# apache/incubator-predictionio

Measured on NVIDIA H100. Metric: ALS iterations/sec, higher is better.
Workload: dtype f32

## Files before the change

### incubator-predictionio_b200/csrc/als_pair_kernel.cuh

```cuda
#pragma once
#include <cuda_fp16.h>
#include <cuda_runtime.h>
#include <stdint.h>

#include "als_kernels.cuh"
#include "als_lockstep.cuh"

namespace pio {
namespace pr {

constexpr int KP = 64;
constexpr int CH = 8;
constexpr int RSTR = KP;
constexpr int NSTAGE = 4;
constexpr int STAGE = CH * RSTR;
constexpr int NTILE = 20;
using LL = LsLayout<KP>;
constexpr int SLOT_STRIDE = LL::STRIDE;
constexpr int VSTR = 80;
constexpr int PART_FLOATS = LL::SIZE + KP;
static_assert(NSTAGE * STAGE <= SLOT_STRIDE, "the staging ring lives in the second slot");
static_assert(NSTAGE % 2 == 0, "a loop step consumes two stages");
constexpr int W_BVEC = 2 * SLOT_STRIDE;
constexpr int W_COL = W_BVEC + 2 * VSTR;
constexpr int W_MVAL = W_COL + 2 * VSTR;
constexpr int W_FLOATS = W_MVAL + NSTAGE * CH + 8;
constexpr size_t smem_bytes(int warps) { return sizeof(float) * (size_t)W_FLOATS * warps; }

__device__ __forceinline__ int split_exponent(float vmax) {
  if (!(vmax > 0.f)) return 0;
  if (isinf(vmax)) return -63;
  int x;
  frexpf(vmax, &x);
  const int e = 15 - x;
  return e < -63 ? -63 : e > 63 ? 63 : e;
}
__device__ __forceinline__ float pow2f(int e) { return __int_as_float((127 + e) << 23); }

__global__ void __launch_bounds__(256) abs_max_kernel(const float* __restrict__ x, long long n, unsigned* out) {
  float m = 0.f;
  const long long stride = (long long)gridDim.x * blockDim.x;
  const long long i0 = (long long)blockIdx.x * blockDim.x + threadIdx.x;
  long long tail = 0;
  if ((reinterpret_cast<uintptr_t>(x) & 15) == 0) {
    const long long n4 = n >> 2;
    for (long long i = i0; i < n4; i += stride) {
      const float4 v = __ldg(reinterpret_cast<const float4*>(x) + i);
      m = fmaxf(m, fmaxf(fmaxf(fabsf(v.x), fabsf(v.y)), fmaxf(fabsf(v.z), fabsf(v.w))));
    }
    tail = 4 * n4;
  }
  for (long long i = tail + i0; i < n; i += stride) m = fmaxf(m, fabsf(__ldg(x + i)));
#pragma unroll
  for (int o = 16; o > 0; o >>= 1) m = fmaxf(m, __shfl_xor_sync(0xffffffffu, m, o));
  if ((threadIdx.x & 31) == 0) atomicMax(out, __float_as_uint(m));
}

__device__ __forceinline__ uint64_t pack2(uint32_t x, uint32_t y) {
  uint64_t r;
  asm("mov.b64 %0, {%1, %2};" : "=l"(r) : "r"(x), "r"(y));
  return r;
}
__device__ __forceinline__ void mma_f16_p(float (&d)[4], const uint32_t (&a)[4], uint64_t b) {
  asm volatile(
      "{\n .reg .b32 b0, b1;\n mov.b64 {b0, b1}, %8;\n"
      "mma.sync.aligned.m16n8k16.row.col.f32.f16.f16.f32 {%0,%1,%2,%3}, {%4,%5,%6,%7}, {b0,b1}, {%0,%1,%2,%3};\n}\n"
      : "+f"(d[0]), "+f"(d[1]), "+f"(d[2]), "+f"(d[3])
      : "r"(a[0]), "r"(a[1]), "r"(a[2]), "r"(a[3]), "l"(b));
}
__device__ __forceinline__ void mma_f16_zp(float (&d)[4], const uint32_t (&a)[4], uint64_t b) {
  asm volatile(
      "{\n .reg .b32 b0, b1;\n mov.b64 {b0, b1}, %4;\n"
      "mma.sync.aligned.m16n8k16.row.col.f32.f16.f16.f32 {%0,%1,%2,%3}, {%5,%6,%7,%8}, {b0,b1}, {%9,%9,%9,%9};\n}\n"
      : "=f"(d[0]), "=f"(d[1]), "=f"(d[2]), "=f"(d[3])
      : "l"(b), "r"(a[0]), "r"(a[1]), "r"(a[2]), "r"(a[3]), "f"(0.f));
}

__device__ __forceinline__ void split2(float a, float b, uint32_t& hi, uint32_t& lo) {
  const __half2 h = __floats2half2_rn(a, b);
  const float2 hf = __half22float2(h);
  const __half2 l = __floats2half2_rn(__fsub_rn(a, hf.x), __fsub_rn(b, hf.y));
  hi = *reinterpret_cast<const uint32_t*>(&h);
  lo = *reinterpret_cast<const uint32_t*>(&l);
}

template <bool IMPLICIT>
__device__ __forceinline__ void accumulate_row(const SolveParams& p, long long beg, long long end, float s, float unscale,
                                               const float* __restrict__ yty, float* ring, float* mval, float* slot,
                                               float* bv) {
  const int lane = threadIdx.x & 31;
  const int g = lane >> 2, t = lane & 3;
  const int nchunks = 2 * (int)((end - beg + 2 * CH - 1) / (2 * CH));
  const int prow = lane >> 4, psl = lane & 15;

  int nidx;
  float nval;
  auto prefetch_meta = [&](int c) {
    const long long e = beg + (long long)c * CH + (lane & 15);
    nidx = (c < nchunks && e < end) ? __ldg(p.idx + e) : -1;
    nval = (lane < 2 * CH && c < nchunks && e < end) ? __ldg(p.val + e) : 0.f;
  };
  auto issue = [&](int c) {
    if (c < nchunks) {
#pragma unroll
      for (int h = 0; h < 2; ++h) {
        float* sbuf = ring + ((c + h) % NSTAGE) * STAGE;
#pragma unroll
        for (int j = 0; j < 4; ++j) {
          const int r = 2 * j + prow;
          const int src = __shfl_sync(0xffffffffu, nidx, CH * h + r);
          float4* d4 = reinterpret_cast<float4*>(sbuf + r * RSTR + ((psl * 4) ^ (8 * r)));
          if (src >= 0) cp_async16(d4, p.src + (size_t)src * KP + psl * 4);
          else *d4 = make_float4(0.f, 0.f, 0.f, 0.f);
        }
      }
      if (lane < 2 * CH) mval[(c % NSTAGE) * CH + lane] = nval;
    }
    cp_async_commit();
  };

  float acc[NTILE][4];
#pragma unroll
  for (int i = 0; i < NTILE; ++i)
#pragma unroll
    for (int e = 0; e < 4; ++e) acc[i][e] = 0.f;
  float pb[4][2];
#pragma unroll
  for (int i = 0; i < 4; ++i) pb[i][0] = pb[i][1] = 0.f;

  int xo[4];
#pragma unroll
  for (int q = 0; q < 4; ++q) xo[q] = g + 8 * (q ^ t);

  prefetch_meta(0);
  issue(0);
  prefetch_meta(2);

#pragma unroll 1
  for (int c = 0; c < nchunks; c += 2) {
    cp_async_wait<0>();
    __syncwarp();
    issue(c + 2);
    prefetch_meta(c + 4);
    const float* XA = ring + (c % NSTAGE) * STAGE + t * RSTR;
    const float* XB = XA + STAGE;
    const float* mv = mval + (c % NSTAGE) * CH;
    float wb[4], sc[4];
    {
      const float r[4] = {mv[t], mv[t + 4], mv[CH + t], mv[CH + t + 4]};
#pragma unroll
      for (int q = 0; q < 4; ++q) {
        wb[q] = r[q];
        sc[q] = s;
        if (IMPLICIT) {
          const float c1 = p.alpha * fabsf(r[q]);
          sc[q] = __fmul_rn(sqrtf(c1), s);
          wb[q] = r[q] > 0.f ? 1.f + c1 : 0.f;
        }
      }
    }
    uint32_t hi[4][4], lo[4][4];
#pragma unroll
    for (int i = 0; i < 4; ++i) {
#pragma unroll
      for (int e = 0; e < 2; ++e) {
        const int q = 2 * i + e;
        const int c0 = xo[q & 3] + 32 * (q >> 2), c4 = 4 * RSTR + xo[q & 3] + 32 * (1 - (q >> 2));
        const float a0 = XA[c0], a4 = XA[c4], b0 = XB[c0], b4 = XB[c4];
        pb[i][e] = fmaf(wb[0], a0, pb[i][e]);
        pb[i][e] = fmaf(wb[1], a4, pb[i][e]);
        pb[i][e] = fmaf(wb[2], b0, pb[i][e]);
        pb[i][e] = fmaf(wb[3], b4, pb[i][e]);
        split2(__fmul_rn(a0, sc[0]), __fmul_rn(a4, sc[1]), hi[i][e], lo[i][e]);
        split2(__fmul_rn(b0, sc[2]), __fmul_rn(b4, sc[3]), hi[i][e + 2], lo[i][e + 2]);
      }
    }
#pragma unroll
    for (int j = 0; j < 8; ++j) {
      const int bi = j >> 1, be = j & 1;
      const uint64_t bh = pack2(hi[bi][be], hi[bi][be + 2]), bl = pack2(lo[bi][be], lo[bi][be + 2]);
#pragma unroll
      for (int i = bi; i < 4; ++i) {
        const int tile = i * (i + 1) + j;
        float d[4];
        mma_f16_zp(d, lo[i], bh);
        mma_f16_p(d, hi[i], bl);
        mma_f16_p(d, hi[i], bh);
        acc[tile][0] += d[0];
        acc[tile][1] += d[1];
        acc[tile][2] += d[2];
        acc[tile][3] += d[3];
      }
    }
  }
  cp_async_wait<0>();
  __syncwarp();

#pragma unroll
  for (int i = 0; i < 4; ++i)
#pragma unroll
    for (int e = 0; e < 2; ++e) {
      float v = pb[i][e];
      v += __shfl_xor_sync(0xffffffffu, v, 1);
      v += __shfl_xor_sync(0xffffffffu, v, 2);
      if (t == 0) bv[16 * i + 8 * e + g] = v;
    }
  {
    const float* yl = yty ? yty + g * KP + 2 * t : nullptr;
    int tile = 0;
#pragma unroll
    for (int i = 0; i < 4; ++i) {
#pragma unroll
      for (int j = 0; j <= 2 * i + 1; ++j, ++tile) {
        const int cb = j >> 1;
        const int cc = 8 * (j & 1) + 2 * t;
        float d0 = acc[tile][0] * unscale, d1 = acc[tile][1] * unscale;
        float d2 = acc[tile][2] * unscale, d3 = acc[tile][3] * unscale;
        if (yl) {
          const float2 y0 = __ldg(reinterpret_cast<const float2*>(yl + 16 * i * KP + 8 * j));
          const float2 y1 = __ldg(reinterpret_cast<const float2*>(yl + (16 * i + 8) * KP + 8 * j));
          d0 += y0.x; d1 += y0.y;
          d2 += y1.x; d3 += y1.y;
        }
        if (cb < i) {
          *reinterpret_cast<float2*>(slot + LL::offd(i, cb, g, cc)) = make_float2(d0, d1);
          *reinterpret_cast<float2*>(slot + LL::offd(i, cb, g + 8, cc)) = make_float2(d2, d3);
        } else {
          if (cc <= g) slot[LL::diag(i, g, cc)] = d0;
          if (cc + 1 <= g) slot[LL::diag(i, g, cc + 1)] = d1;
          if (cc <= g + 8) slot[LL::diag(i, g + 8, cc)] = d2;
          if (cc + 1 <= g + 8) slot[LL::diag(i, g + 8, cc + 1)] = d3;
        }
      }
    }
  }
  __syncwarp();
}

__device__ __forceinline__ void fill_identity(float* slot, float* bv) {
  const int lane = threadIdx.x & 31;
  for (int o = lane; o < LL::SIZE; o += 32) slot[o] = 0.f;
  __syncwarp();
  for (int r = lane; r < KP; r += 32) {
    slot[LL::at(r, r)] = 1.f;
    bv[r] = 0.f;
  }
  __syncwarp();
}

template <bool IMPLICIT, int WARPS>
__global__ void __launch_bounds__(32 * WARPS, 12 / WARPS) als_solve_pair_kernel(const SolveParams p, int n_items) {
  extern __shared__ __align__(16) float smem_all[];
  const int warp = threadIdx.x >> 5;
  float* smem = smem_all + warp * W_FLOATS;
  float* slot0 = smem;
  float* slot1 = smem + SLOT_STRIDE;
  float* ring = slot1;
  float* bvec = smem + W_BVEC;
  float* colbuf = smem + W_COL;
  float* mval = smem + W_MVAL;
  const int lane = threadIdx.x & 31;
  const int grp = lane >> 4;
  const int npairs = (n_items + 1) >> 1;
  const float c1_root_max = IMPLICIT ? sqrtf(p.alpha * __uint_as_float(__ldg(p.absmax + 1))) : 1.f;
  const int e = split_exponent(__uint_as_float(__ldg(p.absmax)) * c1_root_max);
  const float s = pow2f(e), unscale = pow2f(-2 * e);

#pragma unroll 1
  for (int base = blockIdx.x * WARPS; base < npairs; base += gridDim.x * WARPS) {
    const int pair = base + warp;
    int row0 = -1, row1 = -1;
    if (pair < npairs) {
#pragma unroll 1
      for (int h = 0; h < 2; ++h) {
        const int item = 2 * pair + h;
        float* slot = h ? slot1 : slot0;
        float* bv = bvec + h * VSTR;
        if (item >= n_items) {
          fill_identity(slot, bv);
          continue;
        }
        long long beg, end;
        if (p.partial) {
          beg = p.wl_beg[item];
          end = p.wl_end[item];
        } else {
          const int r = p.row_begin + item;
          beg = p.ptr[r];
          end = p.ptr[r + 1];
          if (h) row1 = r;
          else row0 = r;
        }
        accumulate_row<IMPLICIT>(p, beg, end, s, unscale, IMPLICIT && !p.partial ? p.yty : nullptr, ring, mval, slot, bv);
        if (p.partial) {
          float* out = p.partial + (size_t)item * PART_FLOATS;
          for (int o = lane; o < LL::SIZE / 4; o += 32)
            reinterpret_cast<float4*>(out)[o] = reinterpret_cast<const float4*>(slot)[o];
          for (int o = lane; o < KP; o += 32) out[LL::SIZE + o] = bv[o];
          __syncwarp();
        }
      }
    }
    if (p.partial) continue;
    if (WARPS > 1) __syncthreads();
    if (pair < npairs) {
      const int myrow = grp ? row1 : row0;
      const int rr = myrow < 0 ? p.row_begin : myrow;
      chol_lockstep<KP>(grp ? slot1 : slot0, bvec + grp * VSTR, p.lambda * p.nreg[rr], p.k, colbuf + grp * VSTR,
                        p.dst + (size_t)(p.dst_row_offset + rr) * KP, myrow >= 0, p.fail);
      __syncwarp();
    }
  }
}

template <bool IMPLICIT>
__global__ void __launch_bounds__(32, 12) als_finish_pair_kernel(const SolveParams p, const int* __restrict__ row_part_ptr,
                                                                  int n_rows) {
  extern __shared__ __align__(16) float smem[];
  float* bvec = smem + W_BVEC;
  float* colbuf = smem + W_COL;
  const int lane = threadIdx.x & 31;
  const int grp = lane >> 4;
  const int npairs = (n_rows + 1) >> 1;
#pragma unroll 1
  for (int pair = blockIdx.x; pair < npairs; pair += gridDim.x) {
#pragma unroll 1
    for (int h = 0; h < 2; ++h) {
      const int r = 2 * pair + h;
      float* slot = smem + h * SLOT_STRIDE;
      float* bv = bvec + h * VSTR;
      if (r >= n_rows) {
        fill_identity(slot, bv);
        continue;
      }
      const int p0 = row_part_ptr[r], p1 = row_part_ptr[r + 1];
      for (int o = lane; o < PART_FLOATS / 4; o += 32) {
        float4 s = make_float4(0.f, 0.f, 0.f, 0.f);
        for (int q = p0; q < p1; ++q) {
          const float4 v = __ldg(reinterpret_cast<const float4*>(p.partial + (size_t)q * PART_FLOATS) + o);
          s.x += v.x; s.y += v.y; s.z += v.z; s.w += v.w;
        }
        if (o < LL::SIZE / 4) reinterpret_cast<float4*>(slot)[o] = s;
        else reinterpret_cast<float4*>(bv)[o - LL::SIZE / 4] = s;
      }
      __syncwarp();
      if (IMPLICIT) {
        ls_add_yty<KP>(slot, p.yty);
        __syncwarp();
      }
    }
    const int myrow = 2 * pair + grp;
    const bool valid = myrow < n_rows;
    const int rr = valid ? myrow : 0;
    chol_lockstep<KP>(smem + grp * SLOT_STRIDE, bvec + grp * VSTR, p.lambda * p.nreg[rr], p.k, colbuf + grp * VSTR,
                      p.dst + (size_t)(p.dst_row_offset + rr) * KP, valid, p.fail);
    __syncwarp();
  }
}

}
}
```

Before: 35.54.

## Stage fp16 hi/lo planes in shared memory and feed MMAs via ldmatrix

Each lane now reads its chunk rows as float4 vectors, computes the weighted b-vector sums and the hi/lo fp16 split for its own columns, then writes the hi and lo halves back over the consumed fp32 stage. The MMA A and B fragments are then loaded with ldmatrix.x4.trans from a swizzled layout. This replaces the scalar per-element shared loads and register packing of the old scheme. The intent is to cut shared-memory load instructions and bank conflicts in the Gram accumulation loop. Missing rows are zero-filled through cp.async src-size instead of a separate store. In exchange it adds extra shared stores and two warp syncs per step, plus more register pressure from the ldmatrix fragments.

```diff
diff --git a/incubator-predictionio_b200/csrc/als_pair_kernel.cuh b/incubator-predictionio_b200/csrc/als_pair_kernel.cuh
--- a/incubator-predictionio_b200/csrc/als_pair_kernel.cuh
+++ b/incubator-predictionio_b200/csrc/als_pair_kernel.cuh
@@ -14,6 +14,8 @@
 constexpr int RSTR = KP;
 constexpr int NSTAGE = 4;
 constexpr int STAGE = CH * RSTR;
+constexpr int PLANE = 2 * CH * KP * 2;
+static_assert(PLANE == STAGE * (int)sizeof(float), "a step's hi and lo planes overwrite its two fp32 stages");
 constexpr int NTILE = 20;
 using LL = LsLayout<KP>;
 constexpr int SLOT_STRIDE = LL::STRIDE;
@@ -56,24 +58,26 @@
   if ((threadIdx.x & 31) == 0) atomicMax(out, __float_as_uint(m));
 }
 
-__device__ __forceinline__ uint64_t pack2(uint32_t x, uint32_t y) {
-  uint64_t r;
-  asm("mov.b64 %0, {%1, %2};" : "=l"(r) : "r"(x), "r"(y));
-  return r;
-}
-__device__ __forceinline__ void mma_f16_p(float (&d)[4], const uint32_t (&a)[4], uint64_t b) {
-  asm volatile(
-      "{\n .reg .b32 b0, b1;\n mov.b64 {b0, b1}, %8;\n"
-      "mma.sync.aligned.m16n8k16.row.col.f32.f16.f16.f32 {%0,%1,%2,%3}, {%4,%5,%6,%7}, {b0,b1}, {%0,%1,%2,%3};\n}\n"
-      : "+f"(d[0]), "+f"(d[1]), "+f"(d[2]), "+f"(d[3])
-      : "r"(a[0]), "r"(a[1]), "r"(a[2]), "r"(a[3]), "l"(b));
-}
-__device__ __forceinline__ void mma_f16_zp(float (&d)[4], const uint32_t (&a)[4], uint64_t b) {
-  asm volatile(
-      "{\n .reg .b32 b0, b1;\n mov.b64 {b0, b1}, %4;\n"
-      "mma.sync.aligned.m16n8k16.row.col.f32.f16.f16.f32 {%0,%1,%2,%3}, {%5,%6,%7,%8}, {b0,b1}, {%9,%9,%9,%9};\n}\n"
-      : "=f"(d[0]), "=f"(d[1]), "=f"(d[2]), "=f"(d[3])
-      : "l"(b), "r"(a[0]), "r"(a[1]), "r"(a[2]), "r"(a[3]), "f"(0.f));
+__device__ __forceinline__ void mma_f16(float (&d)[4], const uint32_t (&a)[4], uint32_t b0, uint32_t b1) {
+  asm volatile("mma.sync.aligned.m16n8k16.row.col.f32.f16.f16.f32 {%0,%1,%2,%3}, {%4,%5,%6,%7}, {%8,%9}, {%0,%1,%2,%3};\n"
+               : "+f"(d[0]), "+f"(d[1]), "+f"(d[2]), "+f"(d[3])
+               : "r"(a[0]), "r"(a[1]), "r"(a[2]), "r"(a[3]), "r"(b0), "r"(b1));
+}
+__device__ __forceinline__ void mma_f16_z(float (&d)[4], const uint32_t (&a)[4], uint32_t b0, uint32_t b1) {
+  asm volatile("mma.sync.aligned.m16n8k16.row.col.f32.f16.f16.f32 {%0,%1,%2,%3}, {%4,%5,%6,%7}, {%8,%9}, {%10,%10,%10,%10};\n"
+               : "=f"(d[0]), "=f"(d[1]), "=f"(d[2]), "=f"(d[3])
+               : "r"(a[0]), "r"(a[1]), "r"(a[2]), "r"(a[3]), "r"(b0), "r"(b1), "f"(0.f));
+}
+__device__ __forceinline__ void ldsm_x4_t(uint32_t (&r)[4], uint32_t saddr) {
+  asm volatile("ldmatrix.sync.aligned.m8n8.x4.trans.shared.b16 {%0,%1,%2,%3}, [%4];\n"
+               : "=r"(r[0]), "=r"(r[1]), "=r"(r[2]), "=r"(r[3])
+               : "r"(saddr)
+               : "memory");
+}
+
+__device__ __forceinline__ void cp_async16_zfill(void* smem_dst, const void* gsrc, bool copy) {
+  const unsigned s = (unsigned)__cvta_generic_to_shared(smem_dst);
+  asm volatile("cp.async.cg.shared.global [%0], [%1], 16, %2;\n" ::"r"(s), "l"(gsrc), "r"(copy ? 16 : 0));
 }
 
 __device__ __forceinline__ void split2(float a, float b, uint32_t& hi, uint32_t& lo) {
@@ -92,6 +96,7 @@
   const int g = lane >> 2, t = lane & 3;
   const int nchunks = 2 * (int)((end - beg + 2 * CH - 1) / (2 * CH));
   const int prow = lane >> 4, psl = lane & 15;
+  auto ring_col = [](int r, int f) { return f ^ (4 * (r & 1) + 8 * (r & 2)); };
 
   int nidx;
   float nval;
@@ -109,9 +114,8 @@
         for (int j = 0; j < 4; ++j) {
           const int r = 2 * j + prow;
           const int src = __shfl_sync(0xffffffffu, nidx, CH * h + r);
-          float4* d4 = reinterpret_cast<float4*>(sbuf + r * RSTR + ((psl * 4) ^ (8 * r)));
-          if (src >= 0) cp_async16(d4, p.src + (size_t)src * KP + psl * 4);
-          else *d4 = make_float4(0.f, 0.f, 0.f, 0.f);
+          cp_async16_zfill(sbuf + r * RSTR + ring_col(r, psl * 4), p.src + (size_t)(src < 0 ? 0 : src) * KP + psl * 4,
+                           src >= 0);
         }
       }
       if (lane < 2 * CH) mval[(c % NSTAGE) * CH + lane] = nval;
@@ -124,13 +128,17 @@
   for (int i = 0; i < NTILE; ++i)
 #pragma unroll
     for (int e = 0; e < 4; ++e) acc[i][e] = 0.f;
-  float pb[4][2];
-#pragma unroll
-  for (int i = 0; i < 4; ++i) pb[i][0] = pb[i][1] = 0.f;
-
-  int xo[4];
-#pragma unroll
-  for (int q = 0; q < 4; ++q) xo[q] = g + 8 * (q ^ t);
+  float pb[8];
+#pragma unroll
+  for (int j = 0; j < 8; ++j) pb[j] = 0.f;
+
+  int wo[2];
+#pragma unroll
+  for (int e = 0; e < 2; ++e) wo[e] = (2 * t + e) * 128 + ((g ^ (2 * t + e)) << 4);
+  const int lm = lane >> 3, lr = lane & 7;
+  const uint32_t offa = (lr + 8 * (lm >> 1)) * 128 + (((lm & 1) ^ lr) << 4);
+  const uint32_t offb = (lr + 8 * (lm & 1)) * 128 + (((lm >> 1) ^ lr) << 4);
+  const uint32_t ring_s = (uint32_t)__cvta_generic_to_shared(ring);
 
   prefetch_meta(0);
   issue(0);
@@ -140,14 +148,25 @@
   for (int c = 0; c < nchunks; c += 2) {
     cp_async_wait<0>();
     __syncwarp();
+    float* X = ring + (c % NSTAGE) * STAGE;
+    const float* mv = mval + (c % NSTAGE) * CH;
+    const float r[4] = {mv[t], mv[t + 4], mv[CH + t], mv[CH + t + 4]};
+    float x[4][8];
+#pragma unroll
+    for (int q = 0; q < 4; ++q)
+#pragma unroll
+      for (int w = 0; w < 2; ++w) {
+        const float4 v = *reinterpret_cast<const float4*>(X + (q >> 1) * STAGE + (t + 4 * (q & 1)) * RSTR +
+                                                          ring_col(t, 8 * g + 4 * w));
+        x[q][4 * w] = v.x;
+        x[q][4 * w + 1] = v.y;
+        x[q][4 * w + 2] = v.z;
+        x[q][4 * w + 3] = v.w;
+      }
     issue(c + 2);
     prefetch_meta(c + 4);
-    const float* XA = ring + (c % NSTAGE) * STAGE + t * RSTR;
-    const float* XB = XA + STAGE;
-    const float* mv = mval + (c % NSTAGE) * CH;
     float wb[4], sc[4];
     {
-      const float r[4] = {mv[t], mv[t + 4], mv[CH + t], mv[CH + t + 4]};
 #pragma unroll
       for (int q = 0; q < 4; ++q) {
         wb[q] = r[q];
@@ -160,36 +179,55 @@
       }
     }
     uint32_t hi[4][4], lo[4][4];
+    {
+#pragma unroll
+      for (int j = 0; j < 8; ++j)
+#pragma unroll
+        for (int q = 0; q < 4; ++q) pb[j] = fmaf(wb[q], x[q][j], pb[j]);
+#pragma unroll
+      for (int q = 0; q < 4; ++q)
+#pragma unroll
+        for (int k = 0; k < 4; ++k)
+          split2(__fmul_rn(x[q][2 * k], sc[q]), __fmul_rn(x[q][2 * k + 1], sc[q]), hi[q][k], lo[q][k]);
+    }
+    __syncwarp();
+    {
+      char* X8 = reinterpret_cast<char*>(X);
+#pragma unroll
+      for (int q = 0; q < 4; ++q) {
+        char* o = X8 + wo[q & 1] + 1024 * (q >> 1);
+        *reinterpret_cast<uint4*>(o) = make_uint4(hi[q][0], hi[q][1], hi[q][2], hi[q][3]);
+        *reinterpret_cast<uint4*>(o + PLANE) = make_uint4(lo[q][0], lo[q][1], lo[q][2], lo[q][3]);
+      }
+    }
+    __syncwarp();
+    const uint32_t hp = ring_s + (c % NSTAGE) * STAGE * (uint32_t)sizeof(float);
+    uint32_t ah[4][4], al[4][4];
 #pragma unroll
     for (int i = 0; i < 4; ++i) {
-#pragma unroll
-      for (int e = 0; e < 2; ++e) {
-        const int q = 2 * i + e;
-        const int c0 = xo[q & 3] + 32 * (q >> 2), c4 = 4 * RSTR + xo[q & 3] + 32 * (1 - (q >> 2));
-        const float a0 = XA[c0], a4 = XA[c4], b0 = XB[c0], b4 = XB[c4];
-        pb[i][e] = fmaf(wb[0], a0, pb[i][e]);
-        pb[i][e] = fmaf(wb[1], a4, pb[i][e]);
-        pb[i][e] = fmaf(wb[2], b0, pb[i][e]);
-        pb[i][e] = fmaf(wb[3], b4, pb[i][e]);
-        split2(__fmul_rn(a0, sc[0]), __fmul_rn(a4, sc[1]), hi[i][e], lo[i][e]);
-        split2(__fmul_rn(b0, sc[2]), __fmul_rn(b4, sc[3]), hi[i][e + 2], lo[i][e + 2]);
-      }
-    }
-#pragma unroll
-    for (int j = 0; j < 8; ++j) {
-      const int bi = j >> 1, be = j & 1;
-      const uint64_t bh = pack2(hi[bi][be], hi[bi][be + 2]), bl = pack2(lo[bi][be], lo[bi][be + 2]);
-#pragma unroll
-      for (int i = bi; i < 4; ++i) {
-        const int tile = i * (i + 1) + j;
-        float d[4];
-        mma_f16_zp(d, lo[i], bh);
-        mma_f16_p(d, hi[i], bl);
-        mma_f16_p(d, hi[i], bh);
-        acc[tile][0] += d[0];
-        acc[tile][1] += d[1];
-        acc[tile][2] += d[2];
-        acc[tile][3] += d[3];
+      ldsm_x4_t(ah[i], hp + (offa ^ (i << 5)));
+      ldsm_x4_t(al[i], hp + PLANE + (offa ^ (i << 5)));
+    }
+#pragma unroll
+    for (int bi = 0; bi < 4; ++bi) {
+      uint32_t bh[4], bl[4];
+      ldsm_x4_t(bh, hp + (offb ^ (bi << 5)));
+      ldsm_x4_t(bl, hp + PLANE + (offb ^ (bi << 5)));
+#pragma unroll
+      for (int be = 0; be < 2; ++be) {
+        const int j = 2 * bi + be;
+#pragma unroll
+        for (int i = bi; i < 4; ++i) {
+          const int tile = i * (i + 1) + j;
+          float d[4];
+          mma_f16_z(d, al[i], bh[2 * be], bh[2 * be + 1]);
+          mma_f16(d, ah[i], bl[2 * be], bl[2 * be + 1]);
+          mma_f16(d, ah[i], bh[2 * be], bh[2 * be + 1]);
+          acc[tile][0] += d[0];
+          acc[tile][1] += d[1];
+          acc[tile][2] += d[2];
+          acc[tile][3] += d[3];
+        }
       }
     }
   }
@@ -197,14 +235,12 @@
   __syncwarp();
 
 #pragma unroll
-  for (int i = 0; i < 4; ++i)
-#pragma unroll
-    for (int e = 0; e < 2; ++e) {
-      float v = pb[i][e];
-      v += __shfl_xor_sync(0xffffffffu, v, 1);
-      v += __shfl_xor_sync(0xffffffffu, v, 2);
-      if (t == 0) bv[16 * i + 8 * e + g] = v;
-    }
+  for (int j = 0; j < 8; ++j) {
+    float v = pb[j];
+    v += __shfl_xor_sync(0xffffffffu, v, 1);
+    v += __shfl_xor_sync(0xffffffffu, v, 2);
+    if (t == 0) bv[8 * g + j] = v;
+  }
   {
     const float* yl = yty ? yty + g * KP + 2 * t : nullptr;
     int tile = 0;
```

New measurement: 36.40, median of 6. +2.4%, better.
